# lauraset/Super-resolution-building-height-estimation

Measured on AMD Instinct MI355X. Metric: tiles/sec (64x64x8ch->256x256 height), higher is better.
Workload: dtype f16 operands / f32 accumulate (MFMA), f32 residual stream; 1 GPU; RRDBNet x4 (23 RRDB, 64 feat) forward_feature, batch 32 tiles/GPU, 64x64x3 -> 64x256x256 (BASELINE.json configs[1]); global_batch=32, parallelism=tile-sharded x1 (no data-path collective)

## Files before the change

super-resolution-building-height-estimation_amd/csrc/srbh_aux.hip:

```cpp
#include "srbh_internal.h"

namespace srbh {

static thread_local char g_err[512] = "";

unsigned long long g_path_counters[PATH_N] = {};
void set_error(const char* fmt, ...) {
    va_list ap;
    va_start(ap, fmt);
    vsnprintf(g_err, sizeof(g_err), fmt, ap);
    va_end(ap);
}

int hip_fail(hipError_t e, const char* what) {
    set_error("HIP error %d (%s) in %s", (int)e, hipGetErrorString(e), what);
    return (int)e;
}

__global__ void zero_words_kernel(unsigned* __restrict__ p, size_t n) {
    size_t i = (size_t)blockIdx.x * blockDim.x + threadIdx.x;
    const size_t stride = (size_t)gridDim.x * blockDim.x;
    for (; i < n; i += stride) p[i] = 0u;
}

// ... 138 lines not shown
    float acc[8] = {0.f, 0.f, 0.f, 0.f, 0.f, 0.f, 0.f, 0.f};
    for (long px = (long)blockIdx.x * 64 + pl; px < npix; px += (long)gridDim.x * 64) {
        const int x = (int)(px % W);
        const long r = px / W;
        const int y = (int)(r % H), b = (int)(r / H);
        const uint4 v = *(const uint4*)(src + (long)b * img_b + (long)chunk * plane_b + (long)(y + 1) * row_b + (x + 1) * PIX_B + oct * 16);
        const unsigned w4[4] = {v.x, v.y, v.z, v.w};
#pragma unroll
        for (int k = 0; k < 4; ++k) {
            if constexpr (BF) {
                acc[2 * k] += __builtin_bit_cast(float, w4[k] << 16);
                acc[2 * k + 1] += __builtin_bit_cast(float, w4[k] & 0xffff0000u);
            } else {
                acc[2 * k] += (float)__builtin_bit_cast(_Float16, (unsigned short)(w4[k] & 0xffffu));
                acc[2 * k + 1] += (float)__builtin_bit_cast(_Float16, (unsigned short)(w4[k] >> 16));
            }
        }
    }
#pragma unroll
    for (int k = 0; k < 8; ++k) {
        float a = acc[k];
#pragma unroll
        for (int m = 4; m < 64; m <<= 1) a += __shfl_xor(a, m);
        if ((threadIdx.x & 63) < 4) atomicAdd(&red[oct * 8 + k], a);
    }
    __syncthreads();
    if (threadIdx.x < 32) atomicAdd(out + chunk * 32 + threadIdx.x, red[threadIdx.x]);
}

template <int CIN, int BF16 = 0>
__global__ __launch_bounds__(256) void conv_first_kernel(const float* __restrict__ x, const float* __restrict__ w,
                                                         const float* __restrict__ bias, int B, int cin_rt, int H, int W,
                                                         float* ra, float* rb, float* rc, char* out16, int row_b,
                                                         int plane_b, long img_b) {
    extern __shared__ float s_w[];
    const int cin = CIN > 0 ? CIN : cin_rt;
    for (int u = threadIdx.x; u < cin * 9 * 64; u += 256) {
        const int oc = u & 63, k = u >> 6;
        s_w[u] = w[(long)oc * cin * 9 + k];
    }
    __syncthreads();
    const int wq = (W + 3) >> 2;
    const long idx = (long)blockIdx.x * 256 + threadIdx.x;
    const long total = (long)B * H * wq * 16;
    if (idx >= total) return;
    const int og = idx & 15;
    long r = idx >> 4;
    const int xg = r % wq; r /= wq;
    const int yy = r % H;
    const int b = r / H;
    const int x0 = xg * 4;
    float acc[4][4];
#pragma unroll
    for (int p = 0; p < 4; ++p)
#pragma unroll
        for (int q = 0; q < 4; ++q) acc[p][q] = bias ? bias[og * 4 + q] : 0.f;
    for (int ic = 0; ic < cin; ++ic) {
        const float* xp = x + ((long)b * cin + ic) * H * W;
#pragma unroll
        for (int ky = 0; ky < 3; ++ky) {
            const int sy = yy + ky - 1;
            float in[6];
#pragma unroll
            for (int j = 0; j < 6; ++j) {
                const int sx = x0 + j - 1;
                in[j] = (sy >= 0 && sy < H && sx >= 0 && sx < W) ? xp[(long)sy * W + sx] : 0.f;
            }
#pragma unroll
            for (int kx = 0; kx < 3; ++kx) {
// ... 241 lines not shown
    return SRBH_OK;
}

extern "C" int srbh_lrelu_bwd_f32(float* g, const float* y, float slope, long n, void* stream) {
    SRBH_REQUIRE(g && y && n > 0 && (n & 3) == 0, "srbh_lrelu_bwd_f32: bad arguments");
    const long n4 = n / 4;
    const int blocks = (int)((n4 + 255) / 256 < 4096 ? (n4 + 255) / 256 : 4096);
    hipLaunchKernelGGL(lrelu_bwd_kernel, dim3(blocks), dim3(256), 0, (hipStream_t)stream, (float4*)g, (const float4*)y, slope, n4);
    SRBH_HIP(hipGetLastError());
    return SRBH_OK;
}

extern "C" int srbh_act16_channel_sum(const void* src, int B, int H, int W, int chunks_total, int chunk0, int nchunk, int bf16, float* out,
                                      void* stream) {
    SRBH_REQUIRE(src && out && B > 0 && H > 0 && W > 0 && nchunk > 0 && chunk0 >= 0 && chunk0 + nchunk <= chunks_total, "srbh_act16_channel_sum: bad arguments");
    const Act16Geo g = act16_geo(B, chunks_total, H, W);
    if (int rc = zero_async(out, (size_t)nchunk * 32 * sizeof(float), (hipStream_t)stream)) return rc;
    const long npix = (long)B * H * W;
    const int gx = (int)((npix + 255) / 256 < 1024 ? (npix + 255) / 256 : 1024);
    const char* base = (const char*)src + (long)chunk0 * g.plane_b;
    if (bf16) hipLaunchKernelGGL(act16_channel_sum_kernel<1>, dim3(gx, nchunk), dim3(256), 0, (hipStream_t)stream, base, B, H, W, nchunk, g.row_b, g.plane_b, g.img_b, out);
    else hipLaunchKernelGGL(act16_channel_sum_kernel<0>, dim3(gx, nchunk), dim3(256), 0, (hipStream_t)stream, base, B, H, W, nchunk, g.row_b, g.plane_b, g.img_b, out);
    SRBH_HIP(hipGetLastError());
    return SRBH_OK;
}

extern "C" int srbh_conv_first_f32(const float* x, const float* w, const float* bias, int B, int cin, int H, int W,
                                   float* ra, float* rb, float* rc, void* out16, int out16_chunks_total,
                                   void* stream) {
    return srbh::conv_first_f32(x, w, bias, B, cin, H, W, ra, rb, rc, out16, out16_chunks_total, 0, stream);
}

int srbh::conv_first_f32(const float* x, const float* w, const float* bias, int B, int cin, int H, int W, float* ra, float* rb, float* rc,
                         void* out16, int out16_chunks_total, int bf16, void* stream) {
    SRBH_REQUIRE(x && w && B > 0 && cin > 0 && H > 0 && W > 0, "srbh_conv_first_f32: bad arguments");
    SRBH_REQUIRE(!out16 || out16_chunks_total >= 2, "srbh_conv_first_f32: out16 needs >= 2 chunk planes");
    Act16Geo g = act16_geo(B, out16_chunks_total > 0 ? out16_chunks_total : 2, H, W);
    SRBH_REQUIRE(cin <= 56, "srbh_conv_first_f32: at most 56 input channels (got %d)", cin);
    long total = (long)B * H * ((W + 3) / 4) * 16;
    const size_t lds = (size_t)cin * 9 * 64 * sizeof(float);
    if (cin == 3 && bf16)
        hipLaunchKernelGGL((conv_first_kernel<3, 1>), dim3((total + 255) / 256), dim3(256), lds, (hipStream_t)stream, x, w, bias,
                           B, cin, H, W, ra, rb, rc, (char*)out16, g.row_b, g.plane_b, g.img_b);
    else if (cin == 3)
        hipLaunchKernelGGL(conv_first_kernel<3>, dim3((total + 255) / 256), dim3(256), lds, (hipStream_t)stream, x, w, bias,
                           B, cin, H, W, ra, rb, rc, (char*)out16, g.row_b, g.plane_b, g.img_b);
    else if (bf16) {
        if (lds > 65536)
            SRBH_ONCE_PER_DEVICE(SRBH_HIP(hipFuncSetAttribute((const void*)conv_first_kernel<0, 1>, hipFuncAttributeMaxDynamicSharedMemorySize, 56 * 9 * 64 * 4)));
        hipLaunchKernelGGL((conv_first_kernel<0, 1>), dim3((total + 255) / 256), dim3(256), lds, (hipStream_t)stream, x, w, bias,
                           B, cin, H, W, ra, rb, rc, (char*)out16, g.row_b, g.plane_b, g.img_b);
    } else {
        if (lds > 65536)
            SRBH_ONCE_PER_DEVICE(SRBH_HIP(hipFuncSetAttribute((const void*)conv_first_kernel<0>, hipFuncAttributeMaxDynamicSharedMemorySize, 56 * 9 * 64 * 4)));
        hipLaunchKernelGGL(conv_first_kernel<0>, dim3((total + 255) / 256), dim3(256), lds, (hipStream_t)stream, x, w, bias,
                           B, cin, H, W, ra, rb, rc, (char*)out16, g.row_b, g.plane_b, g.img_b);
    }
    SRBH_HIP(hipGetLastError());
    return SRBH_OK;
}
```

super-resolution-building-height-estimation_amd/csrc/srbh_internal.h:

```cpp
#pragma once
#include <hip/hip_runtime.h>
#include <stdarg.h>
#include <stdio.h>
#include <vector>
#include "srbh.h"

namespace srbh {

constexpr int PIX_B = 64;
constexpr int CHUNK_C = 32;
constexpr int TILE_W = 64;
constexpr int TILE_H = 8;

void set_error(const char* fmt, ...);
enum PathCounter { PATH_HCONV16 = 0, PATH_HCONV_TEMPLATE, PATH_ENTRY_FUSED, PATH_ENTRY_SPLIT, PATH_WGRAD16, PATH_WGRAD_B16_GENERIC,
                   PATH_WGRAD_F32, PATH_WGRAD_ENTRY_FUSED, PATH_WGRAD_ENTRY_SPLIT, PATH_HCONV_UP, PATH_HBWD16, PATH_HBLOCK16, PATH_N };
extern unsigned long long g_path_counters[PATH_N];
inline void count_path(int i) { ++g_path_counters[i]; }
int zero_async(void* p, size_t bytes, hipStream_t st);
int hip_fail(hipError_t e, const char* what);

#define SRBH_HIP(call)                                         \
    do {                                                       \
        hipError_t e_ = (call);                                \
// ... 9 lines not shown
    } while (0)

#define SRBH_ONCE_PER_DEVICE(stmt)                        \
    do {                                                  \
        static unsigned long long done_ = 0;              \
        int dev_ = 0;                                     \
        SRBH_HIP(hipGetDevice(&dev_));                    \
        if (!((done_ >> (dev_ & 63)) & 1ull)) {           \
            stmt;                                         \
            done_ |= 1ull << (dev_ & 63);                 \
        }                                                 \
    } while (0)

struct Act16Geo {
    int row_b;
    int plane_b;
    long img_b;
    size_t total_b;
};
inline Act16Geo act16_geo(int B, int chunks, int H, int W) {
    Act16Geo g;
    g.row_b = (W + 2) * PIX_B;
    g.plane_b = (H + 2) * g.row_b;
    g.img_b = (long)chunks * g.plane_b;
    size_t slack = (size_t)(TILE_H + 4) * (size_t)((W + 2 > TILE_W + 2) ? (W + 2) : (TILE_W + 2)) * PIX_B + 8192;
    g.total_b = (size_t)B * g.img_b + slack;
    g.total_b = (g.total_b + 255) & ~(size_t)255;
    return g;
}


size_t ptrunk_aux_bytes(int B, int tiles_per_img);
size_t ptrunk_err_offset(int B, int tiles_per_img);
int ptail_run(const srbh_conv3x3_args* a, hipStream_t stream, int* used);
int ptrunk_takes(int num_block, int H, int W, int* takes, int* ncu_out);
int ptrunk_run(const srbh_rrdbnet_desc* d, void* dense0, void* dense1, float* xr, float* xrr, int B, int H, int W,
               void* aux, hipStream_t stream, int* used, int* final_cur, long train_stride = 0, const void* mask = nullptr, long mask_stride = 0,
               bool bf16 = false);
int conv3x3_trunk_b16(const srbh_conv3x3_args* a, int out_f16, void* stream);
int conv_first_f32(const float* x, const float* w, const float* bias, int B, int cin, int H, int W, float* ra, float* rb, float* rc,
                   void* out16, int out16_chunks_total, int bf16, void* stream);


#if defined(__HIP_DEVICE_COMPILE__) || defined(__HIPCC__)
__device__ __forceinline__ void fold_stat_slots(double* stats, const int C, const int clear, double* red, double& s, double& q) {
    constexpr int NS = 64;
    const int t = threadIdx.x, V = 2 * C, G = 256 / V, v = t % V, g = t / V;
    double part = 0.0;
    if (g < G) {
        for (int k = g; k < NS; k += G) part += stats[(long)k * V + v];
        if (clear)
            for (int k = g; k < NS; k += G) stats[(long)k * V + v] = 0.0;
        red[g * V + v] = part;
    }
    __syncthreads();
    s = 0.0;
    q = 0.0;
    if (t < C)
        for (int k = 0; k < G; ++k) {
            s += red[k * V + t];
            q += red[k * V + C + t];
        }
}

__device__ __forceinline__ unsigned bf16x2_rne(float lo, float hi) {
    typedef float f2_t __attribute__((ext_vector_type(2)));
    typedef __bf16 b2_t __attribute__((ext_vector_type(2)));
    const f2_t f = {lo, hi};
    return __builtin_bit_cast(unsigned, __builtin_convertvector(f, b2_t));
}
#endif
}
```

super-resolution-building-height-estimation_amd/csrc/srbh_ptail.hip:

```cpp
#include <stdlib.h>
#include "srbh_conv3x3_kernel.h"

namespace {
using namespace srbh;
using namespace srbh_k;

struct TParams {
    const char* in;
    long in_img_b;
    int in_plane_b, in_row_b;
    const char* w;
    const float* bias;
    int H, W;
    int tiles_x, tiles_per_img, ntiles, tiles_per_wg;
    int lrelu;
    char* out16;
    long out16_img_b;
    int out16_plane_b, out16_row_b;
    int out16_pix_b, out16_border;
    float* out32;
};

constexpr int W_RES_B = 2 * 36 * 1024;

template <int UPS>
__global__ __launch_bounds__(256, 1) void ptail_kernel(const TParams p) {
    using G = TileGeo<UPS>;
    constexpr int IN_EX = G::UNITS * 16;
    constexpr int CB = 2;
    extern __shared__ __attribute__((aligned(16))) char smem[];
    const int tid = threadIdx.x;
    const int lane = tid & 63;
    const int wave = __builtin_amdgcn_readfirstlane(tid >> 6);
    const int l31 = lane & 31, hi = lane >> 5;
    const int wr = wave >> 1, wc = wave & 1;

    int goff[G::NJ];
#pragma unroll
    for (int j = 0; j < G::NJ; ++j) {
        const int u0 = j * 256 + tid;
        const int u = u0 < G::UNITS ? u0 : 0;
        const int trow = u / (G::COLS * 4);
        const int rem = u - trow * (G::COLS * 4);
        const int pc = rem >> 2, ps = rem & 3;
        goff[j] = trow * p.in_row_b + pc * PIX_B + ((ps ^ ((pc >> 2) & 3)) << 4);
    }
    const unsigned long long tail_mask = __builtin_amdgcn_ballot_w64((G::NJ - 1) * 256 + tid < G::UNITS);
    int aoff[3][2];
#pragma unroll
    for (int dx = 0; dx < 3; ++dx) {
        const int pc = UPS ? (((wc * 32 + l31 + dx - 1) >> 1) + 1) : (wc * 32 + l31 + dx);
#pragma unroll
        for (int ks = 0; ks < 2; ++ks)
            aoff[dx][ks] = wr * (UPS ? 2 : 4) * G::ROW_B + pc * PIX_B + (((ks * 2 + hi) ^ ((pc >> 2) & 3)) << 4);
    }

    auto dma16 = [&](const char* gaddr, const unsigned lds_off_v, const unsigned long long mask) {
        unsigned long long sv;
        const unsigned lds_off = __builtin_amdgcn_readfirstlane(lds_off_v);
        asm volatile("s_mov_b64 %0, exec\n\ts_mov_b64 exec, %1\n\ts_mov_b32 m0, %2\n\ts_nop 0\n\t"
                     "global_load_lds_dwordx4 %3, off\n\ts_mov_b64 exec, %0"
                     : "=&s"(sv) : "s"(mask), "s"(lds_off), "v"(gaddr) : "memory", "m0");
    };
    auto tile_origin = [&](int t, int& img, int& Y0, int& X0) {
        img = t / p.tiles_per_img;
        const int trem = t - img * p.tiles_per_img;
        const int ty = trem / p.tiles_x;
        Y0 = ty * TILE_H;
        X0 = (trem - ty * p.tiles_x) * TILE_W;
    };
    auto stage_inputs = [&](int t) {
        int img, Y0, X0;
        tile_origin(t, img, Y0, X0);
        const char* src0 = p.in + (long)img * p.in_img_b + (long)(UPS ? (Y0 >> 1) : Y0) * p.in_row_b + (UPS ? (X0 >> 1) : X0) * PIX_B;
#pragma unroll
        for (int c = 0; c < 2; ++c)
#pragma unroll
            for (int j = 0; j < G::NJ; ++j)
                dma16(src0 + (long)c * p.in_plane_b + goff[j], W_RES_B + c * IN_EX + (j * 256 + wave * 64) * 16,
                      j < G::NJ - 1 ? ~0ull : tail_mask);
    };

    const int nst = ((p.H & (TILE_H - 1)) == 0 && (p.W & (TILE_W - 1)) == 0) ? (p.out32 ? 32 : 0) + (p.out16 ? 16 : 0) : 0;
    const int t0 = blockIdx.x * p.tiles_per_wg;
    const int t1 = (t0 + p.tiles_per_wg < p.ntiles) ? t0 + p.tiles_per_wg : p.ntiles;
    if (t0 >= t1) return;
#pragma unroll
    for (int k = 0; k < 18; ++k) dma16(p.w + (wave + 4 * k) * 1024 + lane * 16, (wave + 4 * k) * 1024, ~0ull);
    stage_inputs(t0);
    floatx4 bias4[CB][4];
#pragma unroll
    for (int mb = 0; mb < CB; ++mb)
#pragma unroll
        for (int g = 0; g < 4; ++g)
            bias4[mb][g] = p.bias ? *(const floatx4*)(p.bias + mb * 32 + g * 8 + hi * 4) : floatx4{0.f, 0.f, 0.f, 0.f};

    for (int t = t0; t < t1; ++t) {
        int img, Y0, X0;
        tile_origin(t, img, Y0, X0);
        if (t == t0 || nst == 0) asm volatile("s_waitcnt vmcnt(0)" ::: "memory");
        else if (nst == 16) asm volatile("s_waitcnt vmcnt(16)" ::: "memory");
        else if (nst == 32) asm volatile("s_waitcnt vmcnt(32)" ::: "memory");
        else asm volatile("s_waitcnt vmcnt(48)" ::: "memory");
        __syncthreads();
        floatx16 acc[CB][4];
#pragma unroll
        for (int mb = 0; mb < CB; ++mb)
#pragma unroll
            for (int i = 0; i < 4; ++i)
#pragma unroll
                for (int r = 0; r < 16; ++r) acc[mb][i][r] = 0.f;
        constexpr int NREAD = G::NP + 3 * CB, NMFMA = 12 * CB;
        half8 P[2][G::NP];
        half8 A[2][3][CB];
        auto load_group = [&](int q, int set) {
            const int c = q / 6, g = q - c * 6;
            const int ks = g / 3, dx = g - ks * 3;
            const char* sbi = smem + W_RES_B + c * IN_EX;
            const char* sbw = smem + c * (36 * 1024) + lane * 16;
// ... 18 lines not shown
                    for (int mb = 0; mb < CB; ++mb)
                        acc[mb][i] = __builtin_amdgcn_mfma_f32_32x32x16_f16(A[q & 1][dy][mb], P[q & 1][pr], acc[mb][i], 0, 0, 0);
                }
            if (q == 0) __builtin_amdgcn_sched_group_barrier(0x100, NREAD, 0);
            if (q + 1 < 12) {
#pragma unroll
                for (int k = 0; k < NREAD; ++k) {
                    __builtin_amdgcn_sched_group_barrier(0x008, 1, 0);
                    __builtin_amdgcn_sched_group_barrier(0x100, 1, 0);
                }
                __builtin_amdgcn_sched_group_barrier(0x008, NMFMA - NREAD, 0);
            } else {
                __builtin_amdgcn_sched_group_barrier(0x008, NMFMA, 0);
            }
        }
        __syncthreads();
        if (t + 1 < t1) stage_inputs(t + 1);

        const int X = X0 + wc * 32 + l31;
#pragma unroll
        for (int i = 0; i < 4; ++i) {
            const int Y = Y0 + wr * 4 + i;
            const bool valid = (Y < p.H) && (X < p.W);
            const long pix = ((long)img * p.H + Y) * p.W + X;
#pragma unroll
            for (int mb = 0; mb < CB; ++mb) {
                unsigned hp[4][2];
#pragma unroll
                for (int g = 0; g < 4; ++g) {
                    floatx4 v;
#pragma unroll
                    for (int q = 0; q < 4; ++q) v[q] = acc[mb][i][g * 4 + q];
                    v += bias4[mb][g];
                    if (p.lrelu) {
#pragma unroll
                        for (int q = 0; q < 4; ++q) v[q] = v[q] >= 0.f ? v[q] : v[q] * 0.2f;
                    }
                    if (p.out32 && valid) *(floatx4*)(p.out32 + pix * 64 + mb * 32 + g * 8 + hi * 4) = v;
                    half4 h4;
#pragma unroll
                    for (int q = 0; q < 4; ++q) h4[q] = (_Float16)v[q];
                    const uint2 u = __builtin_bit_cast(uint2, h4);
                    hp[g][0] = u.x;
                    hp[g][1] = u.y;
                }
                if (p.out16) {
#pragma unroll
                    for (int m = 0; m < 2; ++m) {
                        auto s0 = __builtin_amdgcn_permlane32_swap(hp[2 * m][0], hp[2 * m + 1][0], false, false);
                        auto s1 = __builtin_amdgcn_permlane32_swap(hp[2 * m][1], hp[2 * m + 1][1], false, false);
                        typedef unsigned uintx4 __attribute__((ext_vector_type(4)));
                        const uintx4 raw = {s0[0], s1[0], s0[1], s1[1]};
                        if (valid)
                            *(uintx4*)(p.out16 + (long)img * p.out16_img_b + (long)mb * p.out16_plane_b + (long)(Y + p.out16_border) * p.out16_row_b +
                                       (X + p.out16_border) * p.out16_pix_b + m * 32 + hi * 16) = raw;
                    }
                }
            }
        }
    }
}

thread_local int g_ptail_wgs_cap = 0;

template <int UPS>
int launch(const TParams& p0, hipStream_t stream) {
    constexpr int LDS_B = W_RES_B + 2 * TileGeo<UPS>::UNITS * 16;
    static_assert(LDS_B <= 163840, "resident weights + both input chunks must fit the 160 KiB LDS");
    SRBH_ONCE_PER_DEVICE(SRBH_HIP(hipFuncSetAttribute((const void*)ptail_kernel<UPS>, hipFuncAttributeMaxDynamicSharedMemorySize, LDS_B)));
    static int ncu_of[64] = {0};
    int dev = 0;
    SRBH_HIP(hipGetDevice(&dev));
    if (!ncu_of[dev & 63]) SRBH_HIP(hipDeviceGetAttribute(&ncu_of[dev & 63], hipDeviceAttributeMultiprocessorCount, dev));
    int ncu = ncu_of[dev & 63];
    if (g_ptail_wgs_cap > 0 && g_ptail_wgs_cap < ncu) ncu = g_ptail_wgs_cap;
    if (const char* we = getenv("SRBH_PTAIL_WGS")) {
        const int cap = atoi(we);
        if (cap > 0 && cap < ncu_of[dev & 63]) ncu = cap;
    }
    TParams p = p0;
    const int nwg = p.ntiles < ncu ? p.ntiles : ncu;
    p.tiles_per_wg = (p.ntiles + nwg - 1) / nwg;
    const int grid = (p.ntiles + p.tiles_per_wg - 1) / p.tiles_per_wg;
    hipLaunchKernelGGL(ptail_kernel<UPS>, dim3(grid), dim3(256), LDS_B, stream, p);
    SRBH_HIP(hipGetLastError());
    return SRBH_OK;
}

}

extern "C" int srbh_ptail_wgs_cap(int cap) {
    const int prev = g_ptail_wgs_cap;
    g_ptail_wgs_cap = cap > 0 ? cap : 0;
    return prev;
}

namespace srbh {

int ptail_run(const srbh_conv3x3_args* a, hipStream_t stream, int* used) {
    *used = 0;
    const char* e = getenv("SRBH_PTAIL");
    if (e && e[0] == '0') return SRBH_OK;
    if (a->in_chunks != 2 || a->cout != 64 || a->res1 || a->res2 || a->skip) return SRBH_OK;
    if (a->out32 && a->out32_c != 64) return SRBH_OK;
    const int tiles_x = (a->W + TILE_W - 1) / TILE_W, tiles_y = (a->H + TILE_H - 1) / TILE_H;
    if (a->out16_nhwc && (!a->out16 || a->out32)) return SRBH_OK;
    if ((long)tiles_x * tiles_y * a->B < 512 && !a->out16_nhwc) return SRBH_OK;
    const int inH = a->upsample2x ? a->H / 2 : a->H, inW = a->upsample2x ? a->W / 2 : a->W;
    const Act16Geo gi = act16_geo(a->B, a->in_chunks_total, inH, inW);
    TParams p{};
    p.in = (const char*)a->in + (long)a->in_chunk0 * gi.plane_b;
    p.in_img_b = gi.img_b;
    p.in_plane_b = gi.plane_b;
    p.in_row_b = gi.row_b;
    p.w = (const char*)a->w;
    p.bias = a->bias;
    p.H = a->H;
    p.W = a->W;
    p.tiles_x = tiles_x;
    p.tiles_per_img = tiles_x * tiles_y;
    p.ntiles = p.tiles_per_img * a->B;
    p.lrelu = a->lrelu;
    if (a->out16 && a->out16_nhwc) {
        const int C = a->out16_chunks_total * 32;
        p.out16 = (char*)a->out16 + (long)a->out16_chunk0 * 64;
        p.out16_pix_b = C * 2;
        p.out16_row_b = a->W * C * 2;
        p.out16_img_b = (long)a->H * a->W * C * 2;
        p.out16_plane_b = 64;
        p.out16_border = 0;
    } else if (a->out16) {
        const Act16Geo go = act16_geo(a->B, a->out16_chunks_total, a->H, a->W);
        p.out16_pix_b = PIX_B;
        p.out16_border = 1;
        p.out16 = (char*)a->out16 + (long)a->out16_chunk0 * go.plane_b;
        p.out16_img_b = go.img_b;
        p.out16_plane_b = go.plane_b;
        p.out16_row_b = go.row_b;
    }
    p.out32 = a->out32;
    const int rc = a->upsample2x ? launch<1>(p, stream) : launch<0>(p, stream);
    if (rc == SRBH_OK) *used = 1;
    return rc;
}

}
```

super-resolution-building-height-estimation_amd/csrc/srbh_ptrunk.hip:

```cpp
#include <stdlib.h>
#include <string.h>
#include <mutex>
#include "srbh_conv3x3_kernel.h"


namespace {
using namespace srbh;
using namespace srbh_k;

struct PLayer {
    const char* w;
    const float* bias;
};

struct PParams {
    char* dense[2];
    long img_b;
    int plane_b, row_b;
    float* xr;
    float* xrr;
    const PLayer* layers;
    int nlayers;
    int H, W, tiles_per_img, nblocks;
    int* prog;
// ... 13 lines not shown
constexpr int IN_EX = G::UNITS * 16;
constexpr int A_STAGE_B = IN_EX + 18 * 1024, B_STAGE_B = IN_EX + 36 * 1024;
constexpr int A_BASE = IN_EX;
constexpr int A_BIAS_OFF = A_BASE + 2 * A_STAGE_B, B_BIAS_OFF = 2 * B_STAGE_B;
constexpr int P_WORD_OFF = A_BIAS_OFF + 128;
constexpr int P_LDS_B = 163840;
static_assert(P_WORD_OFF + 4 <= P_LDS_B && B_BIAS_OFF + 256 <= P_WORD_OFF, "LDS map must fit 160 KiB");
__device__ __forceinline__ int stage_off(int cb, int idx) { return cb == 1 ? A_BASE + idx * A_STAGE_B : idx * B_STAGE_B; }

#include "srbh_ptrunk3_kernel.h"

}

namespace srbh {

unsigned long long* g_ptrunk_prof = nullptr;
static int g_trunk_timing = 0;
static hipEvent_t g_trunk_ev[2];
static int g_trunk_ev_recorded = 0;
static const char* g_trunk_kernel = "none";

constexpr int MAX_BLOCKS = 64;
static size_t table_bytes() { return ((size_t)MAX_BLOCKS * 15 * sizeof(PLayer) + 255) & ~(size_t)255; }
static size_t prog_bytes(int B, int tpi) { return ((size_t)B * 2 * tpi * sizeof(int) + 255) & ~(size_t)255; }

size_t ptrunk_aux_bytes(int B, int tiles_per_img) { return table_bytes() + 2 * prog_bytes(B, tiles_per_img) + 256; }
__global__ void ptrunk_reset_kernel(int* __restrict__ prog, int* __restrict__ xcc, int* __restrict__ err, int n) {
    const int i = blockIdx.x * blockDim.x + threadIdx.x;
    if (i < n) { prog[i] = 0; xcc[i] = 0; }
    if (i == 0) *err = 0;
}

size_t ptrunk_err_offset(int B, int tiles_per_img) { return table_bytes() + prog_bytes(B, tiles_per_img); }

struct TabEntry {
    int dev;
    std::vector<char> host;
    PLayer* dptr;
};
static std::mutex g_tab_mu;
static std::vector<TabEntry> g_tabs;

static int device_table(const std::vector<PLayer>& tab, PLayer** out) {
    int dev = 0;
    SRBH_HIP(hipGetDevice(&dev));
    const size_t nb = tab.size() * sizeof(PLayer);
    std::lock_guard<std::mutex> lock(g_tab_mu);
    for (size_t i = 0; i < g_tabs.size(); ++i)
        if (g_tabs[i].dev == dev && g_tabs[i].host.size() == nb && memcmp(g_tabs[i].host.data(), tab.data(), nb) == 0) {
            *out = g_tabs[i].dptr;
            return SRBH_OK;
        }
    if (g_tabs.size() >= 16) {
        SRBH_HIP(hipFree(g_tabs.front().dptr));
        g_tabs.erase(g_tabs.begin());
    }
    TabEntry e;
    e.dev = dev;
    e.host.assign((const char*)tab.data(), (const char*)tab.data() + nb);
    SRBH_HIP(hipMalloc(&e.dptr, nb));
    SRBH_HIP(hipMemcpy(e.dptr, tab.data(), nb, hipMemcpyHostToDevice));
    *out = e.dptr;
    g_tabs.push_back(std::move(e));
    return SRBH_OK;
}

int ptrunk_takes(int num_block, int H, int W, int* takes, int* ncu_out) {
    *takes = 0;
    if (W != TILE_W || (H % TILE_H) != 0 || num_block <= 0 || num_block > MAX_BLOCKS) return SRBH_OK;
    int dev = 0;
    SRBH_HIP(hipGetDevice(&dev));
    int ncu = 0;
    SRBH_HIP(hipDeviceGetAttribute(&ncu, hipDeviceAttributeMultiprocessorCount, dev));
    if (ncu_out) *ncu_out = ncu;
    if (H / TILE_H > ncu) return SRBH_OK;
    constexpr int LDS_B = P_LDS_B;
    SRBH_ONCE_PER_DEVICE({
        SRBH_HIP(hipFuncSetAttribute((const void*)ptrunk3_kernel<0>, hipFuncAttributeMaxDynamicSharedMemorySize, LDS_B));
        SRBH_HIP(hipFuncSetAttribute((const void*)ptrunk3_kernel<1>, hipFuncAttributeMaxDynamicSharedMemorySize, LDS_B));
        SRBH_HIP(hipFuncSetAttribute((const void*)ptrunk3_kernel<0, 1>, hipFuncAttributeMaxDynamicSharedMemorySize, LDS_B));
        SRBH_HIP(hipFuncSetAttribute((const void*)ptrunk3_kernel<0, 0, 1>, hipFuncAttributeMaxDynamicSharedMemorySize, LDS_B));
    });
    int per_cu = 0;
    SRBH_HIP(hipOccupancyMaxActiveBlocksPerMultiprocessor(&per_cu, ptrunk3_kernel<0>, 256, LDS_B));
    if (per_cu < 1) return SRBH_OK;
    *takes = 1;
    return SRBH_OK;
}

int ptrunk_run(const srbh_rrdbnet_desc* d, void* dense0, void* dense1, float* xr, float* xrr, int B, int H, int W,
               void* aux, hipStream_t stream, int* used, int* final_cur, long train_stride, const void* mask, long mask_stride, bool bf16) {
    *used = 0;
    if (mask && train_stride <= 0) return SRBH_OK;
    SRBH_REQUIRE(!bf16 || (train_stride == 0 && !mask), "ptrunk_run: the bf16 form is the inference forward only");
    int ncu = 0, takes = 0;
    if (int rc = ptrunk_takes(d->num_block, H, W, &takes, &ncu)) return rc;
    if (!takes) return SRBH_OK;
    const int tpi = H / TILE_H;
    constexpr int LDS_B = P_LDS_B;
    const int nl = d->num_block * 15;
    std::vector<PLayer> tab(nl);
    int cur = 0, li = 0;
    for (int blk = 0; blk < d->num_block; ++blk)
        for (int r = 0; r < 3; ++r) {
            const srbh_conv_w* cw = d->rdb + (blk * 3 + r) * 5;
            for (int k = 0; k < 5; ++k) tab[li++] = PLayer{(const char*)cw[k].w, cw[k].bias};
            cur ^= 1;
        }
    *final_cur = cur;
    char* a = (char*)aux;
    PLayer* d_tab = nullptr;
    if (int rc = device_table(tab, &d_tab)) return rc;
    int* d_prog = (int*)(a + table_bytes());
    int* d_err = (int*)(a + ptrunk_err_offset(B, tpi));
    int* d_xcc = (int*)(a + ptrunk_err_offset(B, tpi) + 256);
    hipLaunchKernelGGL(ptrunk_reset_kernel, dim3((B * tpi + 255) / 256), dim3(256), 0, stream, d_prog, d_xcc, d_err, B * tpi);
    SRBH_HIP(hipGetLastError());
    const Act16Geo g = act16_geo(B, 6, H, W);
    int imgs_per_launch = ncu / tpi;
    if (const char* ie = getenv("SRBH_PT_IMAGES")) {
        const int cap = atoi(ie);
        if (cap > 0 && cap < imgs_per_launch) {
            const int nl_ = (B + cap - 1) / cap;
            imgs_per_launch = (B + nl_ - 1) / nl_;
        }
    }
    for (int b0 = 0; b0 < B; b0 += imgs_per_launch) {
        const int nb = (B - b0) < imgs_per_launch ? (B - b0) : imgs_per_launch;
        PParams pp;
        pp.dense_stride = train_stride;
        pp.keep_all = pp.out_pixel = train_stride > 0;
        pp.mask = mask ? (const char*)mask + (long)b0 * g.img_b : nullptr;
        pp.mask_stride = mask_stride;
        pp.dense[0] = (char*)dense0 + (long)b0 * g.img_b;
        pp.dense[1] = (train_stride > 0 ? (char*)dense0 + train_stride : (char*)dense1) + (long)b0 * g.img_b;
        pp.img_b = g.img_b;
        pp.plane_b = g.plane_b;
        pp.row_b = g.row_b;
        pp.xr = xr + (long)b0 * H * W * 64;
        pp.xrr = xrr + (long)b0 * H * W * 64;
        pp.layers = d_tab;
        pp.nlayers = nl;
        pp.H = H;
        pp.W = W;
        pp.tiles_per_img = tpi;
        pp.nblocks = nb * tpi;
        pp.prog = d_prog + b0 * tpi;
        pp.err = d_err;
        pp.xcc = d_xcc + b0 * tpi;
        {
// ... 84 lines not shown
```

super-resolution-building-height-estimation_amd/csrc/srbh_rrdbnet.hip:

```cpp
#include <stdlib.h>
#include "srbh_internal.h"

using namespace srbh;

namespace {

struct WsLayout {
    size_t d0, d1, feat, xr, xrr, u2, u3, u4, aux, total;
    size_t u2lo, u3lo;
    size_t dense_b;
};

inline size_t align256(size_t v) { return (v + 255) & ~(size_t)255; }

__global__ __launch_bounds__(256) void poison_on_error_kernel(const int* __restrict__ err, float* __restrict__ out, size_t n) {
    if (__hip_atomic_load(err, __ATOMIC_RELAXED, __HIP_MEMORY_SCOPE_AGENT) == 0) return;
    const float nan = __builtin_nanf("");
    for (size_t i = (size_t)blockIdx.x * blockDim.x + threadIdx.x; i < n; i += (size_t)gridDim.x * blockDim.x) out[i] = nan;
}

__global__ __launch_bounds__(256) void trunk_out_pixel_order_kernel(const float* __restrict__ src, float* __restrict__ dst, long nquads) {
    typedef float f4 __attribute__((ext_vector_type(4)));
    for (long i = (long)blockIdx.x * blockDim.x + threadIdx.x; i < nquads; i += (long)gridDim.x * blockDim.x) {
        const long row = i >> 10;
// ... 44 lines not shown
extern "C" size_t srbh_rrdbnet_workspace_bytes_f16x2(int B, int H, int W, int want_forward) {
    if (B <= 0 || H <= 0 || W <= 0) return 0;
    return ws_layout(B, H, W, want_forward, true).total;
}

extern "C" int srbh_rrdbnet_forward(const srbh_rrdbnet_desc* d, const float* x, float* out, int B, int H, int W,
                                    int want_forward, void* ws, size_t ws_bytes, void* stream) {
    SRBH_REQUIRE(d && x && out && ws, "srbh_rrdbnet_forward: null pointer");
    SRBH_REQUIRE(B > 0 && H > 0 && W > 0, "srbh_rrdbnet_forward: bad geometry B=%d H=%d W=%d", B, H, W);
    SRBH_REQUIRE(d->num_block >= 0 && d->rdb != nullptr, "srbh_rrdbnet_forward: bad descriptor");
    const bool split = d->tail_f16x2 != 0;
    SRBH_REQUIRE(!split || (d->conv_body_lo && d->conv_up1_lo && d->conv_up2_lo && d->conv_hr_lo),
                 "srbh_rrdbnet_forward: the f16x2 mode needs the lo' packs of conv_body, conv_up1, conv_up2 and conv_hr");
    SRBH_REQUIRE(!split || want_forward != 1, "srbh_rrdbnet_forward: the f16x2 mode computes forward_feature only (want_forward 0 or 2)");
    const WsLayout L = ws_layout(B, H, W, want_forward, split);
    if (ws_bytes < L.total) {
        set_error("srbh_rrdbnet_forward: workspace %zu bytes < required %zu", ws_bytes, L.total);
        return SRBH_ERR_WORKSPACE;
    }
    char* base = (char*)ws;
    void* D[2] = {base + L.d0, base + L.d1};
    float* feat = (float*)(base + L.feat);
    float* xr = (float*)(base + L.xr);
    float* xrr = (float*)(base + L.xrr);
    void* U2 = base + L.u2;
    void* U3 = base + L.u3;
    void* U4 = base + L.u4;

    bool bf16 = false;
    if (d->rdb_b16 && d->num_block > 0) {
        const char* env = getenv("SRBH_TRUNK_BF16");
        bf16 = !(env && env[0] == '0');
    }
    int rc = conv_first_f32(x, d->conv_first_w, d->conv_first_b, B, d->num_in_ch, H, W, feat, xr, xrr, D[0], 6, bf16 ? 1 : 0, stream);
    if (rc) return rc;

    srbh_conv3x3_args a;
    int cur = 0;
    int used_persistent = 0;
    {
        if (persistent_wanted()) {
            srbh_rrdbnet_desc dt = *d;
            if (bf16) dt.rdb = d->rdb_b16;
            rc = ptrunk_run(&dt, D[0], D[1], xr, xrr, B, H, W, base + L.aux, (hipStream_t)stream, &used_persistent, &cur, 0, nullptr, 0, bf16);
            if (rc) return rc;
        }
    }
    for (int blk = 0; !used_persistent && blk < d->num_block; ++blk) {
        for (int r = 0; r < 3; ++r) {
            const srbh_conv_w* cw = (bf16 ? d->rdb_b16 : d->rdb) + (blk * 3 + r) * 5;
            for (int k = 0; k < 4; ++k) {
                a = srbh_conv3x3_args{};
                a.in = D[cur]; a.in_chunks_total = 6; a.in_chunk0 = 0; a.in_chunks = 2 + k;
                a.w = cw[k].w; a.bias = cw[k].bias; a.cout = 32;
                a.B = B; a.H = H; a.W = W; a.lrelu = 1;
                a.out16 = D[cur]; a.out16_chunks_total = 6; a.out16_chunk0 = 2 + k;
                if ((rc = bf16 ? conv3x3_trunk_b16(&a, 0, stream) : srbh_conv3x3_f16(&a, stream))) return rc;
            }
            a = srbh_conv3x3_args{};
            a.in = D[cur]; a.in_chunks_total = 6; a.in_chunk0 = 0; a.in_chunks = 6;
            a.w = cw[4].w; a.bias = cw[4].bias; a.cout = 64;
            a.B = B; a.H = H; a.W = W;
            a.res_scale = 0.2f; a.res1 = xr; a.res1_update = 1;
            if (r == 2) { a.res2 = xrr; a.res2_scale = 0.2f; a.res2_update = 1; }
            a.out16 = D[cur ^ 1]; a.out16_chunks_total = 6; a.out16_chunk0 = 0;
            const bool last = blk + 1 == d->num_block && r == 2;
            if ((rc = bf16 ? conv3x3_trunk_b16(&a, last ? 1 : 0, stream) : srbh_conv3x3_f16(&a, stream))) return rc;
            cur ^= 1;
        }
    }
    const int* err_word = (const int*)(base + L.aux + ptrunk_err_offset(B, (H + TILE_H - 1) / TILE_H));
    auto guard = [&](int out_c) -> int {
        if (!used_persistent) return SRBH_OK;
        hipLaunchKernelGGL(poison_on_error_kernel, dim3(1024), dim3(256), 0, (hipStream_t)stream, err_word, out,
                           (size_t)B * 16 * H * W * out_c);
        SRBH_HIP(hipGetLastError());
        return SRBH_OK;
// ... 31 lines not shown
        a = srbh_conv3x3_args{};
        s = srbh_conv3x3_split{};
        a.in = U3; a.in_chunks_total = 2; a.in_chunk0 = 0; a.in_chunks = 2;
        s.in_lo = base + L.u3lo; s.in_lo_chunks_total = 2; s.in_lo_chunk0 = 0;
        a.w = d->conv_hr.w; s.w_lo = d->conv_hr_lo; a.bias = d->conv_hr.bias; a.cout = 64;
        a.B = B; a.H = 4 * H; a.W = 4 * W;
        if (want_forward == 2) { a.out16 = out; a.out16_chunks_total = 2; a.out16_chunk0 = 0; a.out16_nhwc = 1; }
        else { a.out32 = out; a.out32_c = 64; }
        if ((rc = srbh_conv3x3_f16x2(&a, &s, stream))) return rc;
        return guard(want_forward == 2 ? 32 : 64);
    }
    a = srbh_conv3x3_args{};
    a.in = D[cur]; a.in_chunks_total = 6; a.in_chunk0 = 0; a.in_chunks = 2;
    a.w = d->conv_body.w; a.bias = d->conv_body.bias; a.cout = 64;
    a.B = B; a.H = H; a.W = W; a.skip = feat;
    a.out16 = D[cur ^ 1]; a.out16_chunks_total = 6; a.out16_chunk0 = 0;
    if ((rc = srbh_conv3x3_f16(&a, stream))) return rc;
    a = srbh_conv3x3_args{};
    a.in = D[cur ^ 1]; a.in_chunks_total = 6; a.in_chunk0 = 0; a.in_chunks = 2;
    a.w = d->conv_up1.w; a.bias = d->conv_up1.bias; a.cout = 64;
    a.B = B; a.H = 2 * H; a.W = 2 * W; a.upsample2x = 1; a.lrelu = 1;
    a.out16 = U2; a.out16_chunks_total = 2; a.out16_chunk0 = 0;
    if ((rc = srbh_conv3x3_f16(&a, stream))) return rc;
    a = srbh_conv3x3_args{};
    a.in = U2; a.in_chunks_total = 2; a.in_chunk0 = 0; a.in_chunks = 2;
    a.w = d->conv_up2.w; a.bias = d->conv_up2.bias; a.cout = 64;
    a.B = B; a.H = 4 * H; a.W = 4 * W; a.upsample2x = 1; a.lrelu = 1;
    a.out16 = U3; a.out16_chunks_total = 2; a.out16_chunk0 = 0;
    if ((rc = srbh_conv3x3_f16(&a, stream))) return rc;
    a = srbh_conv3x3_args{};
    a.in = U3; a.in_chunks_total = 2; a.in_chunk0 = 0; a.in_chunks = 2;
    a.w = d->conv_hr.w; a.bias = d->conv_hr.bias; a.cout = 64;
    a.B = B; a.H = 4 * H; a.W = 4 * W;
    if (want_forward == 2) {
        a.out16 = out; a.out16_chunks_total = 2; a.out16_chunk0 = 0; a.out16_nhwc = 1;
        if ((rc = srbh_conv3x3_f16(&a, stream))) return rc;
        return guard(32);
    }
    if (!want_forward) {
        a.out32 = out; a.out32_c = 64;
        if ((rc = srbh_conv3x3_f16(&a, stream))) return rc;
        return guard(64);
    }
    a.lrelu = 1;
    a.out16 = U4; a.out16_chunks_total = 2; a.out16_chunk0 = 0;
    if ((rc = srbh_conv3x3_f16(&a, stream))) return rc;
    SRBH_REQUIRE(d->conv_last.w && d->num_out_ch >= 1 && d->num_out_ch <= 32,
                 "srbh_rrdbnet_forward: conv_last needs 1..32 output channels (got %d)", d->num_out_ch);
    a = srbh_conv3x3_args{};
    a.in = U4; a.in_chunks_total = 2; a.in_chunk0 = 0; a.in_chunks = 2;
    a.w = d->conv_last.w; a.bias = d->conv_last.bias; a.cout = 32;
    a.B = B; a.H = 4 * H; a.W = 4 * W;
    a.out32 = out; a.out32_c = d->num_out_ch;
    if ((rc = srbh_conv3x3_f16(&a, stream))) return rc;
    return guard(d->num_out_ch);
}

extern "C" int srbh_rrdbnet_trunk_out(const void* ws, size_t ws_bytes, int num_block, int B, int H, int W, int want_forward, float* out,
                                      void* stream) {
    SRBH_REQUIRE(ws && out && B > 0 && H > 0 && W > 0 && num_block >= 0, "srbh_rrdbnet_trunk_out: bad arguments");
    const WsLayout L = ws_layout(B, H, W, want_forward);
    if (ws_bytes < L.total) {
        set_error("srbh_rrdbnet_trunk_out: workspace %zu bytes < required %zu", ws_bytes, L.total);
        return SRBH_ERR_WORKSPACE;
    }
    const float* xrr = (const float*)((const char*)ws + L.xrr);
    const size_t n = (size_t)B * H * W * 64;
    int fragment = 0;
    if (persistent_wanted()) {
        if (int rc = ptrunk_takes(num_block, H, W, &fragment, nullptr)) return rc;
    }
    if (!fragment) {
        SRBH_HIP(hipMemcpyAsync(out, xrr, n * sizeof(float), hipMemcpyDeviceToDevice, (hipStream_t)stream));
        return SRBH_OK;
    }
// ... 250 lines not shown
```

Baseline: 7968 tiles/s.

## Fold trunk guard reset and NaN poison into first and tail convolutions

The persistent-trunk guard-word reset kernel is folded into conv_first, so block 0 clears progress, xcc and error words, which removes one launch. The tail conv kernel gains FORM template specialisations (f32 out, act16, act16+lrelu, NHWC16, act16+skip) so epilogue branches are resolved at compile time. It also takes the trunk error word and writes NaN outputs itself, replacing the separate guard kernel on the final conv. The skip-add trunk conv can now use the persistent tail kernel as well. This adds more template instantiations and moves error handling into the kernels.

```diff
diff --git a/super-resolution-building-height-estimation_amd/csrc/srbh_aux.hip b/super-resolution-building-height-estimation_amd/csrc/srbh_aux.hip
--- a/super-resolution-building-height-estimation_amd/csrc/srbh_aux.hip
+++ b/super-resolution-building-height-estimation_amd/csrc/srbh_aux.hip
@@ -194,9 +194,13 @@
 __global__ __launch_bounds__(256) void conv_first_kernel(const float* __restrict__ x, const float* __restrict__ w,
                                                          const float* __restrict__ bias, int B, int cin_rt, int H, int W,
                                                          float* ra, float* rb, float* rc, char* out16, int row_b,
-                                                         int plane_b, long img_b) {
+                                                         int plane_b, long img_b, int* clr_prog, int* clr_xcc, int* clr_err, int clr_n) {
     extern __shared__ float s_w[];
     const int cin = CIN > 0 ? CIN : cin_rt;
+    if (clr_n > 0 && blockIdx.x == 0) {
+        for (int u = threadIdx.x; u < clr_n; u += 256) { clr_prog[u] = 0; clr_xcc[u] = 0; }
+        if (threadIdx.x == 0) *clr_err = 0;
+    }
     for (int u = threadIdx.x; u < cin * 9 * 64; u += 256) {
         const int oc = u & 63, k = u >> 6;
         s_w[u] = w[(long)oc * cin * 9 + k];
@@ -504,30 +508,31 @@
 }
 
 int srbh::conv_first_f32(const float* x, const float* w, const float* bias, int B, int cin, int H, int W, float* ra, float* rb, float* rc,
-                         void* out16, int out16_chunks_total, int bf16, void* stream) {
+                         void* out16, int out16_chunks_total, int bf16, void* stream, int* clr_prog, int* clr_xcc, int* clr_err, int clr_n) {
     SRBH_REQUIRE(x && w && B > 0 && cin > 0 && H > 0 && W > 0, "srbh_conv_first_f32: bad arguments");
     SRBH_REQUIRE(!out16 || out16_chunks_total >= 2, "srbh_conv_first_f32: out16 needs >= 2 chunk planes");
     Act16Geo g = act16_geo(B, out16_chunks_total > 0 ? out16_chunks_total : 2, H, W);
     SRBH_REQUIRE(cin <= 56, "srbh_conv_first_f32: at most 56 input channels (got %d)", cin);
+    SRBH_REQUIRE(clr_n <= 0 || (clr_prog && clr_xcc && clr_err), "srbh_conv_first_f32: null guard-word pointer");
     long total = (long)B * H * ((W + 3) / 4) * 16;
     const size_t lds = (size_t)cin * 9 * 64 * sizeof(float);
     if (cin == 3 && bf16)
         hipLaunchKernelGGL((conv_first_kernel<3, 1>), dim3((total + 255) / 256), dim3(256), lds, (hipStream_t)stream, x, w, bias,
-                           B, cin, H, W, ra, rb, rc, (char*)out16, g.row_b, g.plane_b, g.img_b);
+                           B, cin, H, W, ra, rb, rc, (char*)out16, g.row_b, g.plane_b, g.img_b, clr_prog, clr_xcc, clr_err, clr_n);
     else if (cin == 3)
         hipLaunchKernelGGL(conv_first_kernel<3>, dim3((total + 255) / 256), dim3(256), lds, (hipStream_t)stream, x, w, bias,
-                           B, cin, H, W, ra, rb, rc, (char*)out16, g.row_b, g.plane_b, g.img_b);
+                           B, cin, H, W, ra, rb, rc, (char*)out16, g.row_b, g.plane_b, g.img_b, clr_prog, clr_xcc, clr_err, clr_n);
     else if (bf16) {
         if (lds > 65536)
             SRBH_ONCE_PER_DEVICE(SRBH_HIP(hipFuncSetAttribute((const void*)conv_first_kernel<0, 1>, hipFuncAttributeMaxDynamicSharedMemorySize, 56 * 9 * 64 * 4)));
         hipLaunchKernelGGL((conv_first_kernel<0, 1>), dim3((total + 255) / 256), dim3(256), lds, (hipStream_t)stream, x, w, bias,
-                           B, cin, H, W, ra, rb, rc, (char*)out16, g.row_b, g.plane_b, g.img_b);
+                           B, cin, H, W, ra, rb, rc, (char*)out16, g.row_b, g.plane_b, g.img_b, clr_prog, clr_xcc, clr_err, clr_n);
     } else {
         if (lds > 65536)
             SRBH_ONCE_PER_DEVICE(SRBH_HIP(hipFuncSetAttribute((const void*)conv_first_kernel<0>, hipFuncAttributeMaxDynamicSharedMemorySize, 56 * 9 * 64 * 4)));
         hipLaunchKernelGGL(conv_first_kernel<0>, dim3((total + 255) / 256), dim3(256), lds, (hipStream_t)stream, x, w, bias,
-                           B, cin, H, W, ra, rb, rc, (char*)out16, g.row_b, g.plane_b, g.img_b);
-    }
-    SRBH_HIP(hipGetLastError());
-    return SRBH_OK;
-}
+                           B, cin, H, W, ra, rb, rc, (char*)out16, g.row_b, g.plane_b, g.img_b, clr_prog, clr_xcc, clr_err, clr_n);
+    }
+    SRBH_HIP(hipGetLastError());
+    return SRBH_OK;
+}
diff --git a/super-resolution-building-height-estimation_amd/csrc/srbh_internal.h b/super-resolution-building-height-estimation_amd/csrc/srbh_internal.h
--- a/super-resolution-building-height-estimation_amd/csrc/srbh_internal.h
+++ b/super-resolution-building-height-estimation_amd/csrc/srbh_internal.h
@@ -65,14 +65,21 @@
 
 size_t ptrunk_aux_bytes(int B, int tiles_per_img);
 size_t ptrunk_err_offset(int B, int tiles_per_img);
-int ptail_run(const srbh_conv3x3_args* a, hipStream_t stream, int* used);
+int ptail_run(const srbh_conv3x3_args* a, hipStream_t stream, int* used, const int* err = nullptr, int* err_folded = nullptr);
+enum { TAIL_FORM_EPILOGUE = 1,
+       TAIL_FORM_BODY = 2,
+       TAIL_FORM_RESET = 4,
+       TAIL_FORM_POISON = 8 };
+int tail_forms();
+void ptrunk_guard_words(void* aux, int B, int tiles_per_img, int** prog, int** xcc, int** err, int* n);
 int ptrunk_takes(int num_block, int H, int W, int* takes, int* ncu_out);
 int ptrunk_run(const srbh_rrdbnet_desc* d, void* dense0, void* dense1, float* xr, float* xrr, int B, int H, int W,
                void* aux, hipStream_t stream, int* used, int* final_cur, long train_stride = 0, const void* mask = nullptr, long mask_stride = 0,
-               bool bf16 = false);
+               bool bf16 = false, bool reset = true);
 int conv3x3_trunk_b16(const srbh_conv3x3_args* a, int out_f16, void* stream);
 int conv_first_f32(const float* x, const float* w, const float* bias, int B, int cin, int H, int W, float* ra, float* rb, float* rc,
-                   void* out16, int out16_chunks_total, int bf16, void* stream);
+                   void* out16, int out16_chunks_total, int bf16, void* stream, int* clr_prog = nullptr, int* clr_xcc = nullptr,
+                   int* clr_err = nullptr, int clr_n = 0);
 
 
 #if defined(__HIP_DEVICE_COMPILE__) || defined(__HIPCC__)
diff --git a/super-resolution-building-height-estimation_amd/csrc/srbh_ptail.hip b/super-resolution-building-height-estimation_amd/csrc/srbh_ptail.hip
--- a/super-resolution-building-height-estimation_amd/csrc/srbh_ptail.hip
+++ b/super-resolution-building-height-estimation_amd/csrc/srbh_ptail.hip
@@ -19,13 +19,23 @@
     int out16_plane_b, out16_row_b;
     int out16_pix_b, out16_border;
     float* out32;
+    const float* skip;
+    const int* err;
 };
 
+enum { F_GENERIC = 0, F_F32, F_ACT16, F_ACT16_LRELU, F_NHWC16, F_ACT16_SKIP };
+
 constexpr int W_RES_B = 2 * 36 * 1024;
 
-template <int UPS>
+template <int UPS, int FORM = F_GENERIC>
 __global__ __launch_bounds__(256, 1) void ptail_kernel(const TParams p) {
     using G = TileGeo<UPS>;
+    constexpr bool GEN = FORM == F_GENERIC;
+    constexpr bool REC16 = FORM == F_ACT16 || FORM == F_ACT16_LRELU || FORM == F_ACT16_SKIP;
+    const bool lrelu = GEN ? p.lrelu != 0 : FORM == F_ACT16_LRELU;
+    const bool has32 = GEN ? p.out32 != nullptr : FORM == F_F32;
+    const bool has16 = GEN ? p.out16 != nullptr : FORM != F_F32;
+    const int pix16_b = REC16 ? PIX_B : p.out16_pix_b, border16 = REC16 ? 1 : p.out16_border;
     constexpr int IN_EX = G::UNITS * 16;
     constexpr int CB = 2;
     extern __shared__ __attribute__((aligned(16))) char smem[];
@@ -81,10 +91,34 @@
                       j < G::NJ - 1 ? ~0ull : tail_mask);
     };
 
-    const int nst = ((p.H & (TILE_H - 1)) == 0 && (p.W & (TILE_W - 1)) == 0) ? (p.out32 ? 32 : 0) + (p.out16 ? 16 : 0) : 0;
+    const int nst = ((p.H & (TILE_H - 1)) == 0 && (p.W & (TILE_W - 1)) == 0) ? (has32 ? 32 : 0) + (has16 ? 16 : 0) : 0;
     const int t0 = blockIdx.x * p.tiles_per_wg;
     const int t1 = (t0 + p.tiles_per_wg < p.ntiles) ? t0 + p.tiles_per_wg : p.ntiles;
     if (t0 >= t1) return;
+    if constexpr (FORM == F_F32 || FORM == F_NHWC16) {
+        if (p.err && __hip_atomic_load(p.err, __ATOMIC_RELAXED, __HIP_MEMORY_SCOPE_AGENT) != 0) {
+            typedef unsigned uintx4 __attribute__((ext_vector_type(4)));
+            const uintx4 nanw = {0x7fc00000u, 0x7fc00000u, 0x7fc00000u, 0x7fc00000u};
+            for (int t = t0; t < t1; ++t) {
+                int img, Y0, X0;
+                tile_origin(t, img, Y0, X0);
+                const int X = X0 + wc * 32 + l31;
+                for (int i = 0; i < 4; ++i) {
+                    const int Y = Y0 + wr * 4 + i;
+                    if (Y >= p.H || X >= p.W) continue;
+                    if constexpr (FORM == F_F32) {
+                        const long pix = ((long)img * p.H + Y) * p.W + X;
+                        for (int k = 0; k < 8; ++k) *(uintx4*)(p.out32 + pix * 64 + k * 8 + hi * 4) = nanw;
+                    } else {
+                        for (int k = 0; k < 4; ++k)
+                            *(uintx4*)(p.out16 + (long)img * p.out16_img_b + (long)(k >> 1) * p.out16_plane_b + (long)(Y + border16) * p.out16_row_b +
+                                       (X + border16) * pix16_b + (k & 1) * 32 + hi * 16) = nanw;
+                    }
+                }
+            }
+            return;
+        }
+    }
 #pragma unroll
     for (int k = 0; k < 18; ++k) dma16(p.w + (wave + 4 * k) * 1024 + lane * 16, (wave + 4 * k) * 1024, ~0ull);
     stage_inputs(t0);
@@ -169,19 +203,34 @@
 #pragma unroll
                     for (int q = 0; q < 4; ++q) v[q] = acc[mb][i][g * 4 + q];
                     v += bias4[mb][g];
-                    if (p.lrelu) {
-#pragma unroll
-                        for (int q = 0; q < 4; ++q) v[q] = v[q] >= 0.f ? v[q] : v[q] * 0.2f;
-                    }
-                    if (p.out32 && valid) *(floatx4*)(p.out32 + pix * 64 + mb * 32 + g * 8 + hi * 4) = v;
-                    half4 h4;
-#pragma unroll
-                    for (int q = 0; q < 4; ++q) h4[q] = (_Float16)v[q];
-                    const uint2 u = __builtin_bit_cast(uint2, h4);
-                    hp[g][0] = u.x;
-                    hp[g][1] = u.y;
-                }
-                if (p.out16) {
+                    if constexpr (FORM == F_ACT16_SKIP) {
+                        if (valid) v += *(const floatx4*)(p.skip + pix * 64 + mb * 32 + g * 8 + hi * 4);
+                    }
+                    if constexpr (GEN) {
+                        if (lrelu) {
+#pragma unroll
+                            for (int q = 0; q < 4; ++q) v[q] = v[q] >= 0.f ? v[q] : v[q] * 0.2f;
+                        }
+                    } else if (lrelu) {
+#pragma unroll
+                        for (int q = 0; q < 4; ++q) v[q] = __builtin_fmaxf(v[q], v[q] * 0.2f);
+                    }
+                    if (has32 && valid) *(floatx4*)(p.out32 + pix * 64 + mb * 32 + g * 8 + hi * 4) = v;
+                    if constexpr (GEN) {
+                        half4 h4;
+#pragma unroll
+                        for (int q = 0; q < 4; ++q) h4[q] = (_Float16)v[q];
+                        const uint2 u = __builtin_bit_cast(uint2, h4);
+                        hp[g][0] = u.x;
+                        hp[g][1] = u.y;
+                    } else if (has16) {
+                        typedef float floatx2 __attribute__((ext_vector_type(2)));
+                        typedef _Float16 half2v __attribute__((ext_vector_type(2)));
+                        hp[g][0] = __builtin_bit_cast(unsigned, __builtin_convertvector(floatx2{v[0], v[1]}, half2v));
+                        hp[g][1] = __builtin_bit_cast(unsigned, __builtin_convertvector(floatx2{v[2], v[3]}, half2v));
+                    }
+                }
+                if (has16) {
 #pragma unroll
                     for (int m = 0; m < 2; ++m) {
                         auto s0 = __builtin_amdgcn_permlane32_swap(hp[2 * m][0], hp[2 * m + 1][0], false, false);
@@ -189,8 +238,8 @@
                         typedef unsigned uintx4 __attribute__((ext_vector_type(4)));
                         const uintx4 raw = {s0[0], s1[0], s0[1], s1[1]};
                         if (valid)
-                            *(uintx4*)(p.out16 + (long)img * p.out16_img_b + (long)mb * p.out16_plane_b + (long)(Y + p.out16_border) * p.out16_row_b +
-                                       (X + p.out16_border) * p.out16_pix_b + m * 32 + hi * 16) = raw;
+                            *(uintx4*)(p.out16 + (long)img * p.out16_img_b + (long)mb * p.out16_plane_b + (long)(Y + border16) * p.out16_row_b +
+                                       (X + border16) * pix16_b + m * 32 + hi * 16) = raw;
                     }
                 }
             }
@@ -200,11 +249,11 @@
 
 thread_local int g_ptail_wgs_cap = 0;
 
-template <int UPS>
+template <int UPS, int FORM>
 int launch(const TParams& p0, hipStream_t stream) {
     constexpr int LDS_B = W_RES_B + 2 * TileGeo<UPS>::UNITS * 16;
     static_assert(LDS_B <= 163840, "resident weights + both input chunks must fit the 160 KiB LDS");
-    SRBH_ONCE_PER_DEVICE(SRBH_HIP(hipFuncSetAttribute((const void*)ptail_kernel<UPS>, hipFuncAttributeMaxDynamicSharedMemorySize, LDS_B)));
+    SRBH_ONCE_PER_DEVICE(SRBH_HIP(hipFuncSetAttribute((const void*)ptail_kernel<UPS, FORM>, hipFuncAttributeMaxDynamicSharedMemorySize, LDS_B)));
     static int ncu_of[64] = {0};
     int dev = 0;
     SRBH_HIP(hipGetDevice(&dev));
@@ -219,7 +268,7 @@
     const int nwg = p.ntiles < ncu ? p.ntiles : ncu;
     p.tiles_per_wg = (p.ntiles + nwg - 1) / nwg;
     const int grid = (p.ntiles + p.tiles_per_wg - 1) / p.tiles_per_wg;
-    hipLaunchKernelGGL(ptail_kernel<UPS>, dim3(grid), dim3(256), LDS_B, stream, p);
+    hipLaunchKernelGGL((ptail_kernel<UPS, FORM>), dim3(grid), dim3(256), LDS_B, stream, p);
     SRBH_HIP(hipGetLastError());
     return SRBH_OK;
 }
@@ -234,15 +283,34 @@
 
 namespace srbh {
 
-int ptail_run(const srbh_conv3x3_args* a, hipStream_t stream, int* used) {
+int tail_forms() {
+    const char* e = getenv("SRBH_TAIL_FORMS");
+    return (e && e[0]) ? atoi(e) : TAIL_FORM_EPILOGUE | TAIL_FORM_RESET | TAIL_FORM_POISON;
+}
+
+int ptail_run(const srbh_conv3x3_args* a, hipStream_t stream, int* used, const int* err, int* err_folded) {
     *used = 0;
+    if (err_folded) *err_folded = 0;
     const char* e = getenv("SRBH_PTAIL");
     if (e && e[0] == '0') return SRBH_OK;
-    if (a->in_chunks != 2 || a->cout != 64 || a->res1 || a->res2 || a->skip) return SRBH_OK;
+    if (a->in_chunks != 2 || a->cout != 64 || a->res1 || a->res2) return SRBH_OK;
     if (a->out32 && a->out32_c != 64) return SRBH_OK;
     const int tiles_x = (a->W + TILE_W - 1) / TILE_W, tiles_y = (a->H + TILE_H - 1) / TILE_H;
     if (a->out16_nhwc && (!a->out16 || a->out32)) return SRBH_OK;
-    if ((long)tiles_x * tiles_y * a->B < 512 && !a->out16_nhwc) return SRBH_OK;
+    const int forms = tail_forms();
+    const long ntiles = (long)tiles_x * tiles_y * a->B;
+    int form = F_GENERIC;
+    if (a->skip) {
+        if (!(forms & TAIL_FORM_BODY) || a->upsample2x || a->lrelu || a->out32 || !a->out16 || a->out16_nhwc || ntiles < 256) return SRBH_OK;
+        form = F_ACT16_SKIP;
+    } else {
+        if (ntiles < 512 && !a->out16_nhwc) return SRBH_OK;
+        if (forms & TAIL_FORM_EPILOGUE) {
+            if (a->out32 && !a->out16) form = (a->lrelu || a->upsample2x) ? F_GENERIC : F_F32;
+            else if (a->out16 && !a->out32 && a->out16_nhwc) form = (a->lrelu || a->upsample2x) ? F_GENERIC : F_NHWC16;
+            else if (a->out16 && !a->out32) form = a->lrelu ? F_ACT16_LRELU : a->upsample2x ? F_GENERIC : F_ACT16;
+        }
+    }
     const int inH = a->upsample2x ? a->H / 2 : a->H, inW = a->upsample2x ? a->W / 2 : a->W;
     const Act16Geo gi = act16_geo(a->B, a->in_chunks_total, inH, inW);
     TParams p{};
@@ -276,7 +344,20 @@
         p.out16_row_b = go.row_b;
     }
     p.out32 = a->out32;
-    const int rc = a->upsample2x ? launch<1>(p, stream) : launch<0>(p, stream);
+    p.skip = a->skip;
+    if (err && err_folded && (forms & TAIL_FORM_POISON) && (form == F_F32 || (form == F_NHWC16 && a->out16_chunks_total == 2))) {
+        p.err = err;
+        *err_folded = 1;
+    }
+    int rc;
+    if (a->upsample2x) rc = form == F_ACT16_LRELU ? launch<1, F_ACT16_LRELU>(p, stream) : launch<1, F_GENERIC>(p, stream);
+    else if (form == F_F32) rc = launch<0, F_F32>(p, stream);
+    else if (form == F_ACT16) rc = launch<0, F_ACT16>(p, stream);
+    else if (form == F_ACT16_LRELU) rc = launch<0, F_ACT16_LRELU>(p, stream);
+    else if (form == F_NHWC16) rc = launch<0, F_NHWC16>(p, stream);
+    else if (form == F_ACT16_SKIP) rc = launch<0, F_ACT16_SKIP>(p, stream);
+    else rc = launch<0, F_GENERIC>(p, stream);
+    if (rc != SRBH_OK && err_folded) *err_folded = 0;
     if (rc == SRBH_OK) *used = 1;
     return rc;
 }
diff --git a/super-resolution-building-height-estimation_amd/csrc/srbh_ptrunk.hip b/super-resolution-building-height-estimation_amd/csrc/srbh_ptrunk.hip
--- a/super-resolution-building-height-estimation_amd/csrc/srbh_ptrunk.hip
+++ b/super-resolution-building-height-estimation_amd/csrc/srbh_ptrunk.hip
@@ -69,6 +69,13 @@
 }
 
 size_t ptrunk_err_offset(int B, int tiles_per_img) { return table_bytes() + prog_bytes(B, tiles_per_img); }
+void ptrunk_guard_words(void* aux, int B, int tiles_per_img, int** prog, int** xcc, int** err, int* n) {
+    char* a = (char*)aux;
+    *prog = (int*)(a + table_bytes());
+    *err = (int*)(a + ptrunk_err_offset(B, tiles_per_img));
+    *xcc = (int*)(a + ptrunk_err_offset(B, tiles_per_img) + 256);
+    *n = B * tiles_per_img;
+}
 
 struct TabEntry {
     int dev;
@@ -126,7 +133,8 @@
 }
 
 int ptrunk_run(const srbh_rrdbnet_desc* d, void* dense0, void* dense1, float* xr, float* xrr, int B, int H, int W,
-               void* aux, hipStream_t stream, int* used, int* final_cur, long train_stride, const void* mask, long mask_stride, bool bf16) {
+               void* aux, hipStream_t stream, int* used, int* final_cur, long train_stride, const void* mask, long mask_stride, bool bf16,
+               bool reset) {
     *used = 0;
     if (mask && train_stride <= 0) return SRBH_OK;
     SRBH_REQUIRE(!bf16 || (train_stride == 0 && !mask), "ptrunk_run: the bf16 form is the inference forward only");
@@ -148,11 +156,12 @@
     char* a = (char*)aux;
     PLayer* d_tab = nullptr;
     if (int rc = device_table(tab, &d_tab)) return rc;
-    int* d_prog = (int*)(a + table_bytes());
-    int* d_err = (int*)(a + ptrunk_err_offset(B, tpi));
-    int* d_xcc = (int*)(a + ptrunk_err_offset(B, tpi) + 256);
-    hipLaunchKernelGGL(ptrunk_reset_kernel, dim3((B * tpi + 255) / 256), dim3(256), 0, stream, d_prog, d_xcc, d_err, B * tpi);
-    SRBH_HIP(hipGetLastError());
+    int *d_prog, *d_err, *d_xcc, nwords;
+    ptrunk_guard_words(a, B, tpi, &d_prog, &d_xcc, &d_err, &nwords);
+    if (reset) {
+        hipLaunchKernelGGL(ptrunk_reset_kernel, dim3((nwords + 255) / 256), dim3(256), 0, stream, d_prog, d_xcc, d_err, nwords);
+        SRBH_HIP(hipGetLastError());
+    }
     const Act16Geo g = act16_geo(B, 6, H, W);
     int imgs_per_launch = ncu / tpi;
     if (const char* ie = getenv("SRBH_PT_IMAGES")) {
diff --git a/super-resolution-building-height-estimation_amd/csrc/srbh_rrdbnet.hip b/super-resolution-building-height-estimation_amd/csrc/srbh_rrdbnet.hip
--- a/super-resolution-building-height-estimation_amd/csrc/srbh_rrdbnet.hip
+++ b/super-resolution-building-height-estimation_amd/csrc/srbh_rrdbnet.hip
@@ -100,7 +100,12 @@
         const char* env = getenv("SRBH_TRUNK_BF16");
         bf16 = !(env && env[0] == '0');
     }
-    int rc = conv_first_f32(x, d->conv_first_w, d->conv_first_b, B, d->num_in_ch, H, W, feat, xr, xrr, D[0], 6, bf16 ? 1 : 0, stream);
+    const int forms = tail_forms();
+    const bool fold_reset = persistent_wanted() && d->num_block > 0 && (forms & TAIL_FORM_RESET);
+    int *g_prog = nullptr, *g_xcc = nullptr, *g_err = nullptr, g_n = 0;
+    if (fold_reset) ptrunk_guard_words(base + L.aux, B, (H + TILE_H - 1) / TILE_H, &g_prog, &g_xcc, &g_err, &g_n);
+    int rc = conv_first_f32(x, d->conv_first_w, d->conv_first_b, B, d->num_in_ch, H, W, feat, xr, xrr, D[0], 6, bf16 ? 1 : 0, stream, g_prog, g_xcc,
+                            g_err, g_n);
     if (rc) return rc;
 
     srbh_conv3x3_args a;
@@ -110,7 +115,8 @@
         if (persistent_wanted()) {
             srbh_rrdbnet_desc dt = *d;
             if (bf16) dt.rdb = d->rdb_b16;
-            rc = ptrunk_run(&dt, D[0], D[1], xr, xrr, B, H, W, base + L.aux, (hipStream_t)stream, &used_persistent, &cur, 0, nullptr, 0, bf16);
+            rc = ptrunk_run(&dt, D[0], D[1], xr, xrr, B, H, W, base + L.aux, (hipStream_t)stream, &used_persistent, &cur, 0, nullptr, 0, bf16,
+                            !fold_reset);
             if (rc) return rc;
         }
     }
@@ -208,15 +214,20 @@
     a.in = U3; a.in_chunks_total = 2; a.in_chunk0 = 0; a.in_chunks = 2;
     a.w = d->conv_hr.w; a.bias = d->conv_hr.bias; a.cout = 64;
     a.B = B; a.H = 4 * H; a.W = 4 * W;
+    auto last_conv = [&](int out_c) -> int {
+        int used = 0, folded = 0;
+        if (int rc_ = ptail_run(&a, (hipStream_t)stream, &used, used_persistent ? err_word : nullptr, &folded)) return rc_;
+        if (!used)
+            if (int rc_ = srbh_conv3x3_f16(&a, stream)) return rc_;
+        return folded ? SRBH_OK : guard(out_c);
+    };
     if (want_forward == 2) {
         a.out16 = out; a.out16_chunks_total = 2; a.out16_chunk0 = 0; a.out16_nhwc = 1;
-        if ((rc = srbh_conv3x3_f16(&a, stream))) return rc;
-        return guard(32);
+        return last_conv(32);
     }
     if (!want_forward) {
         a.out32 = out; a.out32_c = 64;
-        if ((rc = srbh_conv3x3_f16(&a, stream))) return rc;
-        return guard(64);
+        return last_conv(64);
     }
     a.lrelu = 1;
     a.out16 = U4; a.out16_chunks_total = 2; a.out16_chunk0 = 0;
```

Result: no change. 8007 tiles/s, median of 6 (+0.5%).
